# aa5490/Distributed-Training-with-Pipeline-Parallelism

Hardware: AMD Instinct MI355X
Metric: tokens/sec/node + pipeline bubble fraction, GPT-2 PP=1/2/4/8 (GPipe vs 1F1B vs interleaved) (higher is better)
Workload: dtype bf16

## Files before the change

csrc/bindings.cpp:

```cpp
#include <climits>
#include <torch/extension.h>
#include <c10/hip/HIPStream.h>
#include <hip/hip_runtime.h>

#include <algorithm>
#include <cstdint>

extern "C" {
int mp_norm_fwd(int f32, int rms, const void* a, const void* b, const void* w, const void* bias, void* s_out, void* y,
                float* mean, float* rstd, int rows, int D, float eps, float p, uint64_t seed, hipStream_t st);
int mp_norm_bwd(int f32, int rms, const void* dy, const void* s, const void* w, const float* mean, const float* rstd,
                const void* dres, void* ds, void* dbranch, float* dw, float* dbias, float* cs_res, float* cs_ds,
                int rows, int D, float p, uint64_t seed, float* part, hipStream_t st);
int64_t mp_norm_bwd_part_elems(int rows, int D);
int64_t mp_colsum_part_elems(int rows, int cols);
int mp_xent_fwd_bwd(void* logits, const int64_t* target, float* loss, int T, int V, int Vp, float grad_scale,
                    int64_t ignore_index, int write_grad, int f32, hipStream_t st);
int mp_embed_fwd(const int64_t* idx, const void* wte, const void* wpe, void* out, int T, int S, int D, int pos_offset,
                 int f32, hipStream_t st);
int mp_embed_bwd(const int64_t* idx, const void* dout, float* dwte, float* dwpe, int T, int S, int D, int pos_offset,
                 int f32, hipStream_t st);
int mp_sumsq(const float* g, int64_t n, float* out, hipStream_t st);
int mp_scaled_sum(const float* x, int64_t n, float scale, float* out, hipStream_t st);
int mp_gemm_f32(const float* A, const float* B, float* C, const float* bias, int M, int N, int K, int64_t lda,
// ... 35 lines not shown
int mp_doc_bounds(const int64_t* tokens, int64_t eos, int* doc_start, int* doc_end, int B, int S, hipStream_t st);
int mp_attn_decode(const void* q, const void* k, const void* v, const int* lens, void* o, float* ws, int B, int H,
                   int Hkv, int D, int Smax, int max_len, int64_t q_stride, int64_t k_bs, int64_t k_ts, int64_t v_bs,
                   int64_t v_ts, int64_t o_stride, float scale, int splits, hipStream_t st);
int mp_attn_decode_plan(int B, int Hkv, int max_len);
int64_t mp_attn_decode_ws_floats(int B, int H, int D, int splits);
int mp_attn_f32_fwd(const float* q, const float* k, const float* v, float* o, float* lse, int B, int Sq, int Sk, int H,
                    int Hkv, int D, int64_t qs, int64_t ks, int64_t vs, int64_t os, int causal, float scale,
                    float p_drop, uint64_t seed, hipStream_t st);
int mp_attn_f32_bwd(const float* q, const float* k, const float* v, const float* o, const float* dout,
                    const float* lse, float* delta, float* dq, float* dk, float* dv, int B, int Sq, int Sk, int H,
                    int Hkv, int D, int64_t qs, int64_t ks, int64_t vs, int64_t os, int64_t dqs, int64_t dks,
                    int64_t dvs, int causal, float scale, float p_drop, uint64_t seed, hipStream_t st);
int mp_set_drop_step_attn_f32(uint64_t v, hipStream_t st);
int mp_set_drop_step_gemm_f32(uint64_t v, hipStream_t st);
int mp_gemm_f32_set_lanes(int lanes);
int mp_transpose(const void* in, void* out, int R, int C, int64_t ldi, int64_t ldo, hipStream_t st);
int mp_transpose_batched(const void* src, void* dst, const int64_t* desc, const int* tile0, int n, int total_tiles,
                         hipStream_t st);
int mp_set_drop_step_attn(uint64_t v, hipStream_t st);
int mp_set_drop_step_elem(uint64_t v, hipStream_t st);
int mp_set_drop_step_norm(uint64_t v, hipStream_t st);
int mp_set_drop_step_gemm(uint64_t v, hipStream_t st);
int mp_gemm2(const void* A, const void* B, void* C, const void* bias, const void* residual, void* aux, int M, int N,
             int K, int64_t lda, int64_t ldb, int64_t ldc, int64_t ld_res, int64_t ld_aux, int transA, int transB,
             int epilogue, int c_f32_accum, float alpha, int force_cfg, float* ws, float* colsum, float p_drop,
             uint64_t seed, hipStream_t st);
int mp_gemm2_plan(int M, int N, int K, int transA, int transB, int c_f32_accum, int force_cfg, int* split_out);
int64_t mp_gemm2_ws_floats(int cfg, int split, int M, int N, int K);
int mp_gemm2_has_probe_engines();
int mp_gemm_tt_grouped(int n, const void* const* A, const void* const* B, float* const* C, const int* M, const int* N,
                       const int* K, const int64_t* lda, const int64_t* ldb, const int64_t* ldc, float alpha,
                       hipStream_t st);
int mp_probe_spin(unsigned* flag, unsigned expect, int64_t timeout_us, unsigned* result, hipStream_t waiter);
int mp_probe_set(unsigned* flag, unsigned value, hipStream_t setter);
int mp_probe_clock_khz();
int mp_gemm(const void* A, const void* B, void* C, const void* bias, const void* residual, void* aux, int M, int N,
            int K, int64_t lda, int64_t ldb, int64_t ldc, int64_t ld_res, int64_t ld_aux, int transA, int transB,
            int epilogue, int c_f32_accum, float alpha, hipStream_t st);
}

namespace {

hipStream_t cur_stream() { return c10::hip::getCurrentHIPStream().stream(); }

void check(int rc, const char* what) { TORCH_CHECK(rc == 0, "mipipe kernel ", what, " failed with code ", rc); }

const void* ptr_or_null(const c10::optional<torch::Tensor>& t) { return t.has_value() ? t->data_ptr() : nullptr; }

int storage(const torch::Tensor& t, const char* name) {
  TORCH_CHECK(t.scalar_type() == torch::kBFloat16 || t.scalar_type() == torch::kFloat32, name,
              " must be bf16 or f32, got ", t.scalar_type());
  return t.scalar_type() == torch::kFloat32 ? 1 : 0;
}
void* mptr_or_null(const c10::optional<torch::Tensor>& t) { return t.has_value() ? t->data_ptr() : nullptr; }

void req(const torch::Tensor& t, torch::ScalarType dt, const char* name) {
  TORCH_CHECK(t.is_cuda(), name, " must be on the GPU");
  TORCH_CHECK(t.scalar_type() == dt, name, " has wrong dtype ", t.scalar_type());
  TORCH_CHECK(t.is_contiguous(), name, " must be contiguous");
}

void reqn(const torch::Tensor& t, torch::ScalarType dt, int64_t n, const char* name) {
  req(t, dt, name);
  TORCH_CHECK(t.numel() == n, name, " has ", t.numel(), " elements, expected ", n);
}
// ... 544 lines not shown
  }
  if (rc == -2 || rc == -1) return 0;
  check(rc, "gemm2");
  return 1;
}

void gemm_tt_grouped(std::vector<torch::Tensor> dy, std::vector<torch::Tensor> x, std::vector<torch::Tensor> C,
                     double alpha) {
  const int n = (int)dy.size();
  TORCH_CHECK(n == (int)x.size() && n == (int)C.size() && n >= 1 && n <= 8, "gemm_tt_grouped: 1..8 problems");
  const void* A[8];
  const void* B[8];
  float* Cp[8];
  int M[8], N[8], K[8];
  int64_t lda[8], ldb[8], ldc[8];
  for (int i = 0; i < n; ++i) {
    TORCH_CHECK(dy[0].is_cuda(), "gemm_tt_grouped: dy must be on the GPU");
    gemm_operand("gemm_tt_grouped", "dy", dy[i], torch::kBFloat16, dy[0]);
    gemm_operand("gemm_tt_grouped", "x", x[i], torch::kBFloat16, dy[0]);
    gemm_operand("gemm_tt_grouped", "C", C[i], torch::kFloat32, dy[0]);
    TORCH_CHECK(dy[i].size(0) == x[i].size(0) && C[i].size(0) == dy[i].size(1) && C[i].size(1) == x[i].size(1),
                "gemm_tt_grouped: shape mismatch");
    A[i] = dy[i].data_ptr();
    B[i] = x[i].data_ptr();
    Cp[i] = C[i].data_ptr<float>();
    M[i] = (int)dy[i].size(1);
    N[i] = (int)x[i].size(1);
    K[i] = (int)dy[i].size(0);
    lda[i] = dy[i].stride(0);
    ldb[i] = x[i].stride(0);
    ldc[i] = C[i].stride(0);
  }
  check(mp_gemm_tt_grouped(n, A, B, Cp, M, N, K, lda, ldb, ldc, (float)alpha, cur_stream()), "gemm_tt_grouped");
}

void transpose(torch::Tensor in, torch::Tensor out) {
  TORCH_CHECK(in.is_cuda() && out.is_cuda() && in.get_device() == out.get_device(), "transpose: in and out must be on one GPU");
  TORCH_CHECK(in.scalar_type() == torch::kBFloat16 && out.scalar_type() == torch::kBFloat16, "transpose: in and out must be bf16");
  TORCH_CHECK(in.dim() == 2 && out.dim() == 2 && in.stride(1) == 1 && out.stride(1) == 1, "transpose: 2-D rows");
  TORCH_CHECK(in.size(0) > 0 && in.size(1) > 0, "transpose: in is empty");
  TORCH_CHECK(out.size(0) == in.size(1) && out.size(1) == in.size(0), "transpose: shape");
  check(mp_transpose(in.data_ptr(), out.data_ptr(), in.size(0), in.size(1), in.stride(0), out.stride(0),
                     cur_stream()),
        "transpose");
}

void transpose_batched(torch::Tensor src, torch::Tensor dst, torch::Tensor desc, torch::Tensor tile0,
                       int64_t total_tiles) {
  TORCH_CHECK(desc.scalar_type() == torch::kInt64 && tile0.scalar_type() == torch::kInt32 && desc.is_cuda() &&
                  tile0.is_cuda() && desc.size(0) == tile0.size(0),
              "transpose_batched: bad descriptors");
  check(mp_transpose_batched(src.data_ptr(), dst.data_ptr(), desc.data_ptr<int64_t>(), tile0.data_ptr<int>(),
                             (int)desc.size(0), (int)total_tiles, cur_stream()),
        "transpose_batched");
}

int64_t create_stream(int64_t device, int64_t priority) {
  int cur = 0;
  TORCH_CHECK(hipGetDevice(&cur) == hipSuccess, "hipGetDevice");
  TORCH_CHECK(hipSetDevice((int)device) == hipSuccess, "hipSetDevice");
  int lo = 0, hi = 0;
  TORCH_CHECK(hipDeviceGetStreamPriorityRange(&lo, &hi) == hipSuccess, "priority range");
  hipStream_t s = nullptr;
  const hipError_t e = hipStreamCreateWithPriority(&s, hipStreamNonBlocking, priority < 0 ? hi : lo);
  hipSetDevice(cur);
  TORCH_CHECK(e == hipSuccess, "hipStreamCreateWithPriority: ", hipGetErrorString(e));
// ... 131 lines not shown
  m.def("embed_bwd", &embed_bwd);
  m.def("sumsq", &sumsq);
  m.def("scaled_sum", &scaled_sum);
  m.def("zero_", &zero_);
  m.def("gemm_f32", &gemm_f32);
  m.def("gemm_f32_set_lanes", &mp_gemm_f32_set_lanes);
  m.def("gemm_f32_ex", &gemm_f32_ex, pybind11::arg("A"), pybind11::arg("B"), pybind11::arg("C"), pybind11::arg("bias"),
        pybind11::arg("R"), pybind11::arg("X"), pybind11::arg("epi") = 0, pybind11::arg("alpha") = 1.0,
        pybind11::arg("accumulate") = false, pybind11::arg("p_drop") = 0.0, pybind11::arg("seed") = 0,
        pybind11::arg("force_ks") = 0);
  m.def("adamw", &adamw);
  m.def("cast_f32_bf16", &cast_f32_bf16);
  m.def("act_fwd", &act_fwd);
  m.def("act_bwd", &act_bwd);
  m.def("colsum", &colsum);
  m.def("swiglu_fwd", &swiglu_fwd);
  m.def("swiglu_bwd", &swiglu_bwd);
  m.def("rope", &rope);
  m.def("attn_fwd", &attn_fwd);
  m.def("attn_bwd", &attn_bwd);
  m.def("attn_doc_fwd", &attn_doc_fwd);
  m.def("attn_doc_bwd", &attn_doc_bwd);
  m.def("doc_bounds", &doc_bounds);
  m.def("attn_decode", &attn_decode, pybind11::arg("q"), pybind11::arg("k_cache"), pybind11::arg("v_cache"),
        pybind11::arg("lens"), pybind11::arg("o"), pybind11::arg("H"), pybind11::arg("Hkv"), pybind11::arg("D"),
        pybind11::arg("max_len"), pybind11::arg("scale"), pybind11::arg("splits") = 0);
  m.def("attn_decode_plan", [](int64_t B, int64_t Hkv, int64_t max_len) {
    return mp_attn_decode_plan((int)B, (int)Hkv, (int)max_len);
  }, "key splits the decode attention picks for B sequences x Hkv KV heads over max_len keys");
  m.def("gemm", &gemm);
  m.def("lane_merge", &lane_merge, pybind11::arg("g0"), pybind11::arg("lanes"), pybind11::arg("sumsq") = pybind11::none());
  m.def("gemm_tt_grouped", &gemm_tt_grouped, pybind11::arg("dy"), pybind11::arg("x"), pybind11::arg("C"),
        pybind11::arg("alpha") = 1.0);
  m.def("gemm2", &gemm2, pybind11::arg("A"), pybind11::arg("B"), pybind11::arg("C"), pybind11::arg("bias"),
        pybind11::arg("residual"), pybind11::arg("aux"), pybind11::arg("transA"), pybind11::arg("transB"),
        pybind11::arg("epilogue"), pybind11::arg("accum"), pybind11::arg("alpha"), pybind11::arg("force_cfg"),
        pybind11::arg("colsum"), pybind11::arg("p_drop") = 0.0, pybind11::arg("seed") = 0);
  m.def("transpose", &transpose);
  m.def("set_dropout_step", &set_dropout_step);
  m.def("create_stream", &create_stream, pybind11::arg("device"), pybind11::arg("priority") = 0);
  m.def("transpose_batched", &transpose_batched);
  m.def("probe_spin", &probe_spin, pybind11::arg("flag"), pybind11::arg("expect"), pybind11::arg("timeout_us"),
        pybind11::arg("result"), pybind11::arg("waiter") = 0);
  m.def("probe_set", &probe_set, pybind11::arg("flag"), pybind11::arg("value"), pybind11::arg("setter") = 0);
  m.def("probe_clock_khz", []() { return mp_probe_clock_khz(); });
  m.def("gemm2_plan", [](int64_t M, int64_t N, int64_t K, bool transA, bool transB, bool accum, int64_t force_cfg) {
    int split = 1;
    const int cfg = mp_gemm2_plan((int)M, (int)N, (int)K, transA, transB, accum, (int)force_cfg, &split);
    return std::make_tuple(cfg, split);
  }, "engine config + split-K factor the v2 GEMM picks (14: stream-K gemm7)");
  m.def("gemm_f32_plan", [](int64_t M, int64_t N, int64_t K, int64_t force_ks) {
    int split = 1, sk_grid = 0, sk_chunk = 0;
    const int big = mp_gemm_f32_plan((int)M, (int)N, (int)K, (int)force_ks, &split, &sk_grid, &sk_chunk);
    return std::make_tuple(big != 0, split, sk_grid, sk_chunk);
  }, "what gemm_f32_ex will run: (128x128 engine, split-K factor, stream-K workgroups, K-tile pairs per workgroup)");
  m.def("gemm2_has_probe_engines", []() { return mp_gemm2_has_probe_engines() != 0; });
}
```

csrc/kernels/gemm2.hip:

```cpp
#include "mp_common.h"

using namespace mp;

typedef __attribute__((ext_vector_type(4))) short s16x4;
typedef __attribute__((ext_vector_type(8))) short s16x8;

#ifndef MP_G3_GROUP
#define MP_G3_GROUP 2
#endif
#ifndef MP_G2_GROUP
#define MP_G2_GROUP 8
#endif

#ifndef MP_G4_SR
#define MP_G4_SR 2
#endif

#ifndef MP_GROUP_MAX
#define MP_GROUP_MAX 8
#endif

namespace g2 {

enum Epi { EPI_NONE = 0, EPI_BIAS = 1, EPI_BIAS_GELU = 2, EPI_BIAS_RELU = 3, EPI_BIAS_RES = 4, EPI_RES = 5,
           EPI_DGELU = 6, EPI_DRELU = 7 };

constexpr int BK = 64;
constexpr int NT = 512;

__device__ __forceinline__ int swz8(int row) { return (((row >> 1) & 1) << 2) | ((row >> 2) & 3); }
__device__ __forceinline__ int swz16(int row) { return ((row & 3) << 2) | ((row >> 2) & 3); }
__device__ __forceinline__ int swzq(int row) { return (((row >> 1) & 7) + 6) & 7; }
// ... 518 lines not shown
        for (int j = 0; j < TN; ++j) bfr[1][j] = frag16<TB, BN>(sbB, wn + 16 * j, 1);
      }
      __builtin_amdgcn_sched_barrier(0);
      __builtin_amdgcn_s_setprio(1);
#pragma unroll
      for (int i = 0; i < TM; ++i)
#pragma unroll
        for (int j = 0; j < TN; ++j) acc[i][j] = mfma16(af[s][i], bfr[s][j], acc[i][j]);
      __builtin_amdgcn_s_setprio(0);
      __builtin_amdgcn_sched_barrier(0);
    }
    }
    asm volatile("s_waitcnt lgkmcnt(0)" ::: "memory");
    __builtin_amdgcn_s_barrier();
    asm volatile("" ::: "memory");
    if (t + 2 < nk) {
      issue(t & 1, t + 2);
      wait_vmcnt<PW>();
    } else {
      wait_vmcnt<0>();
    }
    asm volatile("" ::: "memory");
    __builtin_amdgcn_s_barrier();
    asm volatile("" ::: "memory");
  }

  epilogue<BM, BN, WM, WN, EPI, ACC>(Stage16<TM, TN>{acc, wn, lane}, smem, m0, n0, wr, Cv, bias, R, AUX, WS, M, N, ldc,
                                     ldr, ldx, alpha, nsplit, p_drop, seed);
  }

}


template <int EPI, bool ACC, bool M16, bool TT = false>
__global__ void __launch_bounds__(NT, 1) __attribute__((amdgpu_waves_per_eu(2, 2)))
gemm3_kernel(const bf16_t* __restrict__ A, const bf16_t* __restrict__ B, void* __restrict__ Cv,
             const bf16_t* __restrict__ bias, const bf16_t* __restrict__ R, bf16_t* __restrict__ AUX,
             float* __restrict__ WS, int M, int N, int K, int64_t lda, int64_t ldb, int64_t ldc, int64_t ldr,
             int64_t ldx, float alpha, float p_drop, uint64_t seed, int tile_lim) {
  if (p_drop > 0.f) seed = step_seed(seed);
  constexpr int BM = 256, BN = 256, WM = 2, WN = 4;
  constexpr int HALF = 128 * 128;
  constexpr int BUF = 4 * HALF;
  extern __shared__ __attribute__((aligned(16))) char smem[];

  const int gm = (M + BM - 1) / BM, gn = (N + BN - 1) / BN;
  const int nwg = tile_lim > 0 ? tile_lim : gm * gn;
  int wg, split;
  if (gridDim.y > 1 && tile_lim == 0) {
    const int v = xcd_remap((int)blockIdx.x + (int)gridDim.x * (int)blockIdx.y, nwg * (int)gridDim.y);
    split = v / nwg;
    wg = v % nwg;
  } else {
    wg = xcd_remap((int)blockIdx.x, nwg);
    split = (int)blockIdx.y;
  }
  constexpr int GROUP = MP_G3_GROUP;
  const int group = wg / (GROUP * gn);
  const int first_m = group * GROUP;
  const int gsz = min(gm - first_m, GROUP);
  const int tm = tile_lim > 0 ? wg / gn : first_m + (wg % (GROUP * gn)) % gsz;
  const int tn = tile_lim > 0 ? wg % gn : (wg % (GROUP * gn)) / gsz;
  const int m0 = tm * BM, n0 = tn * BN;

  const int lane = threadIdx.x & 63, hl = lane >> 5, l32 = lane & 31;
  const int wave = __builtin_amdgcn_readfirstlane(threadIdx.x >> 6);
  const int wr = wave / WN, wc = wave % WN;
  const int wm = wr * (BM / WM), wn = wc * (BN / WN);

  const int nsplit = gridDim.y;
  const int ktiles = K / BK;
  const int kt0 = split * ktiles / nsplit;
  const int nk = (split + 1) * ktiles / nsplit - kt0;

  static_assert(!TT || M16, "the TT build exists with 16x16x32 MFMAs only");
  const int lr = lane >> 3;
  const int lc = (lane & 7) ^ (M16 ? swzq(8 * (wave & 1) + lr) : swz8(8 * (wave & 1) + lr));
  const bf16_t* pa[2];
  const bf16_t* pb[2];
  const bf16_t* ta1[2];
  const bf16_t* tb1[2];
  if constexpr (TT) {
    const int kr = lane >> 4;
    const int ic = 8 * ((lane & 15) ^ ((kr << 2) | (wave & 3)));
    const int am = ic < 64 ? ic : ic + 64, bn = 64 * (ic >> 5) + (ic & 31);
    auto cm = [&](int m) { return m < M ? m : M - 8; };
    auto cn = [&](int n) { return n < N ? n : N - 8; };
#pragma unroll
    for (int j = 0; j < 2; ++j) {
      const int64_t krow = (int64_t)kt0 * BK + 4 * wave + 32 * j + kr;
      pa[j] = A + krow * lda + cm(m0 + am);
      ta1[j] = A + krow * lda + cm(m0 + am + 64);
      pb[j] = B + krow * ldb + cn(n0 + bn);
      tb1[j] = B + krow * ldb + cn(n0 + bn + 32);
    }
  }
#pragma unroll
  for (int j = 0; j < 2 && !TT; ++j) {
    int ra = m0 + 128 * j + 8 * wave + lr;
    ra = ra < M ? ra : M - 1;
    int rb = n0 + 64 * ((wave >> 2) + 2 * j) + 8 * (wave & 3) + lr;
    rb = rb < N ? rb : N - 1;
    pa[j] = A + (int64_t)ra * lda + (int64_t)kt0 * BK + lc * 8;
// ... 187 lines not shown
#pragma unroll
      for (int j = 0; j < 2; ++j) b1[j][s_] = fq(buf + 3 * HALF, rB + 16 * j, s_);
    if (t + 1 < nk) issue(3, t + 1);
    if (steady) wait_vmcnt<8>(); else wait_vmcnt<0>();
    G3_BAR();
    asm volatile("s_waitcnt lgkmcnt(0)" ::: "memory");
    G4_MFMA(0, b1, 2);
    G3_BAR();
#pragma unroll
    for (int s_ = 0; s_ < 2; ++s_)
#pragma unroll
      for (int i = 0; i < 4; ++i) af[i][s_] = fq(buf + HALF, rA + 16 * i, s_);
    if (steady) issue(0, t + 2);
    G3_BAR();
    asm volatile("s_waitcnt lgkmcnt(0)" ::: "memory");
    G4_MFMA(4, b0, 0);
    G3_BAR();
    if (steady) {
      issue(1, t + 2);
      wait_vmcnt<8>();
    } else {
      wait_vmcnt<0>();
    }
    G3_BAR();
    G4_MFMA(4, b1, 2);
    G3_BAR();
  }
#undef G4_MFMA
#undef G3_BAR
  if (wr == 0) __builtin_amdgcn_s_barrier();
  __syncthreads();
  epilogue<BM, BN, WM, WN, EPI, ACC>(Stage16<8, 4>{acc, wn, lane}, smem, m0, n0, wr, Cv, bias, R, AUX, WS, M, N, ldc,
                                     ldr, ldx, alpha, nsplit, p_drop, seed, nullptr, 0, 0, split);
  }
}

template <int EPI, bool ACC, bool M16, bool TT = false>
static int launch3(const void* A, const void* B, void* C, const void* bias, const void* R, void* X, float* ws, int M,
                   int N, int K,
                   int64_t lda, int64_t ldb, int64_t ldc, int64_t ldr, int64_t ldx, float alpha, int split,
                   float p_drop, uint64_t seed, hipStream_t st, int tile_lim = 0) {
  constexpr int LDS_MAIN = 2 * 4 * 128 * 128;
  constexpr int EPI_BYTES = 128 * (256 + 4) * 4;
  constexpr int LDS = LDS_MAIN > EPI_BYTES ? LDS_MAIN : EPI_BYTES;
  auto kern = gemm3_kernel<EPI, ACC, M16, TT>;
  static bool attr = false;
  if (!attr) {
    hipFuncSetAttribute((const void*)kern, hipFuncAttributeMaxDynamicSharedMemorySize, LDS);
    attr = true;
  }
  const int nwg = tile_lim > 0 ? tile_lim : ((M + 255) / 256) * ((N + 255) / 256);
  static const bool split_remap = [] {
    const char* e = getenv("MIPIPE_G3_SPLIT_REMAP");
    return e && e[0] == '1';
  }();
  if (tile_lim == 0 && !split_remap) tile_lim = -1;
  kern<<<dim3(nwg, split), NT, LDS, st>>>((const bf16_t*)A, (const bf16_t*)B, C, (const bf16_t*)bias,
                                          (const bf16_t*)R, (bf16_t*)X, ws, M, N, K, lda, ldb, ldc, ldr, ldx, alpha, p_drop, seed,
                                          tile_lim);
  return (int)hipGetLastError();
}

template <int EPI, bool ACC>
__global__ void __launch_bounds__(NT, 1) __attribute__((amdgpu_waves_per_eu(2, 2)))
gemm6_kernel(const bf16_t* __restrict__ A, const bf16_t* __restrict__ B, void* __restrict__ Cv,
             const bf16_t* __restrict__ bias, const bf16_t* __restrict__ R, bf16_t* __restrict__ AUX,
// ... 1270 lines not shown
  int best = 3, best_split = 1;
  float best_t = 3.0e38f;
  const int kt = K / BK;
  for (int c = 0; c < 4; ++c) {
    const int cus = 256;
    const int slots = c == 3 ? 2 * cus : cus;
    if (outer && CFGS[c].bn == 192) continue;
    const int tiles = ((M + CFGS[c].bm - 1) / CFGS[c].bm) * ((N + CFGS[c].bn - 1) / CFGS[c].bn);
    const float area = (float)(CFGS[c].bm * CFGS[c].bn) / (256.f * 256.f) * (c == 3 ? 2.f : 1.f);
    static const int acc_cap = [] {
      const char* e = getenv("MIPIPE_DW_MAXSPLIT");
      const int v = e ? atoi(e) : 32;
      return v > 0 ? v : 32;
    }();
    const int acc_max = kt / 4 < acc_cap ? kt / 4 : acc_cap;
    const int max_split = acc ? acc_max : (kt / 3 < 8 ? kt / 3 : 8);
    for (int s = 1; s <= (max_split > 1 ? max_split : 1); ++s) {
      const int work = tiles * s;
      const int rounds = (work + slots - 1) / slots;
      const int kper = (kt + s - 1) / s;
      const float epi = s > 1 ? (acc ? 6.f : 8.f) : 2.f;
      const float t = rounds * (kper + epi + 2.f) * area / CFGS[c].eff;
      if (t < best_t * 0.999f) {
        best_t = t;
        best = c;
        best_split = s;
      }
    }
  }
  *split_out = best_split;
  return best;
}

}

using namespace g2;

template <bool TA, bool TB, int EPI, bool ACC>
static int dispatch(int cfg, const void* A, const void* B, void* C, const void* bias, const void* R, void* X, float* ws,
                    int M,
                    int N, int K, int64_t lda, int64_t ldb, int64_t ldc, int64_t ldr, int64_t ldx, float alpha,
                    int split, float p_drop, uint64_t seed, hipStream_t st) {
  if constexpr (TA && TB && ACC && EPI == EPI_NONE) {
    if (cfg == 13) return launchs<64, 64, EPI, ACC, true, true>(A, B, C, bias, R, X, ws, M, N, K, lda, ldb, ldc, ldr, ldx, alpha, split, p_drop, seed, st);
    if (cfg == 6) return launch3<EPI, ACC, true, true>(A, B, C, bias, R, X, ws, M, N, K, lda, ldb, ldc, ldr, ldx, alpha, split, p_drop, seed, st);
  }
  if constexpr (!TA && !TB) {
    if (cfg == 10) return launchs<64, 64, EPI, ACC>(A, B, C, bias, R, X, ws, M, N, K, lda, ldb, ldc, ldr, ldx, alpha, split, p_drop, seed, st);
    if (cfg == 11) return launchs<64, 32, EPI, ACC>(A, B, C, bias, R, X, ws, M, N, K, lda, ldb, ldc, ldr, ldx, alpha, split, p_drop, seed, st);
    if (cfg == 12) return launchs<32, 32, EPI, ACC>(A, B, C, bias, R, X, ws, M, N, K, lda, ldb, ldc, ldr, ldx, alpha, split, p_drop, seed, st);
    if (cfg == 4) return launch3<EPI, ACC, false>(A, B, C, bias, R, X, ws, M, N, K, lda, ldb, ldc, ldr, ldx, alpha, split, p_drop, seed, st);
    if (cfg == 5) return launch3<EPI, ACC, true>(A, B, C, bias, R, X, ws, M, N, K, lda, ldb, ldc, ldr, ldx, alpha, split, p_drop, seed, st);
    if (cfg == 9) return launch6<EPI, ACC>(A, B, C, bias, R, X, ws, M, N, K, lda, ldb, ldc, ldr, ldx, alpha, p_drop, seed, st);
    if (cfg == 15) return launch8<EPI, ACC, 2>(A, B, C, bias, R, X, ws, M, N, K, lda, ldb, ldc, ldr, ldx, alpha, p_drop, seed, st);
    if (cfg == 16) return launch8<EPI, ACC, 3>(A, B, C, bias, R, X, ws, M, N, K, lda, ldb, ldc, ldr, ldx, alpha, p_drop, seed, st);
#ifdef MP_PROBE_ENGINES
    if constexpr (!ACC) {
      if (cfg == 8) return launch5<EPI>(A, B, C, bias, R, X, ws, M, N, K, lda, ldb, ldc, ldr, ldx, alpha, p_drop, seed, st);
    }
#endif
  }
  switch (cfg) {
    case 0: return launch<256, 256, 2, 4, TA, TB, EPI, ACC>(A, B, C, bias, R, X, ws, M, N, K, lda, ldb, ldc, ldr, ldx, alpha, split, p_drop, seed, st);
    case 1: return launch<256, 192, 4, 2, TA, TB, EPI, ACC>(A, B, C, bias, R, X, ws, M, N, K, lda, ldb, ldc, ldr, ldx, alpha, split, p_drop, seed, st);
    case 2: return launch<256, 128, 4, 2, TA, TB, EPI, ACC>(A, B, C, bias, R, X, ws, M, N, K, lda, ldb, ldc, ldr, ldx, alpha, split, p_drop, seed, st);
    default: return launch<128, 128, 2, 4, TA, TB, EPI, ACC>(A, B, C, bias, R, X, ws, M, N, K, lda, ldb, ldc, ldr, ldx, alpha, split, p_drop, seed, st);
// ... 267 lines not shown
                                  const int64_t* ldc, float alpha, hipStream_t st) {
  if (n <= 0) return 0;
  if (n > MP_GROUP_MAX) return -1;
  GroupTT g{};
  g.n = n;
  g.alpha = alpha;
  int t = 0;
  for (int i = 0; i < n; ++i) {
    if (M[i] % 8 || N[i] % 8 || K[i] % BK || M[i] <= 0 || N[i] <= 0) return -1;
    g.A[i] = (const bf16_t*)A[i];
    g.B[i] = (const bf16_t*)B[i];
    g.C[i] = C[i];
    g.M[i] = M[i];
    g.N[i] = N[i];
    g.K[i] = K[i];
    g.lda[i] = lda[i];
    g.ldb[i] = ldb[i];
    g.ldc[i] = ldc[i];
    g.tile_start[i] = t;
    t += ((M[i] + 63) / 64) * ((N[i] + 63) / 64);
  }
  for (int i = n; i <= MP_GROUP_MAX; ++i) g.tile_start[i] = t;
  constexpr int STAGE = (64 + 64) * BK * 2;
  constexpr int EPI_BYTES = 32 * (64 + 4) * 4;
  constexpr int LDS = 2 * STAGE > EPI_BYTES ? 2 * STAGE : EPI_BYTES;
  static bool attr = false;
  if (!attr) {
    hipFuncSetAttribute((const void*)gemms_tt_grouped_kernel, hipFuncAttributeMaxDynamicSharedMemorySize, LDS);
    attr = true;
  }
  gemms_tt_grouped_kernel<<<t, 256, LDS, st>>>(g);
  return (int)hipGetLastError();
}
```

distributed-training-with-pipeline-parallelism_amd/models/native.py:

```python
from __future__ import annotations

import contextlib
import hashlib
import os
import math
from dataclasses import dataclass
from typing import Callable, Dict, List, Optional, Sequence, Tuple

import torch

from .. import ops
from .config import NativeConfig



@dataclass
class ParamSpec:
    name: str
    shape: Tuple[int, ...]
    init: str
    decay: bool
    std: float = 0.02
    transpose: bool = False

# ... 426 lines not shown
                wjobs.append(ops.DW(dy, gact, self.g("ffn.w2.weight")))
                if cfg.bias and not fuse_b1:
                    wjobs.append(lambda da=da: ops.colsum(da, self.g("ffn.w1.bias")))
                wjobs.append(ops.DW(da, h2, self.g("ffn.w1.weight")))
                dh2 = ops.linear_dx(da, self.w("ffn.w1.weight"), wt=self.wt("ffn.w1.weight"))
            fuse_cs = cfg.bias and kind == "layernorm"
            dx2, _ = ops.norm_bwd(dh2, st["x2"], self.w("ffn_norm.weight"), st["mu2"], st["rs2"], kind=kind,
                                  dres=dy, dw=self.g("ffn_norm.weight"), dbias=self.gb("ffn_norm.bias"),
                                  colsum_dres=self.g("ffn.w2.bias") if fuse_cs else None,
                                  colsum_ds=self.g("attn.wo.bias") if fuse_cs else None)
            if cfg.bias and not fuse_cs:
                wjobs.append(lambda dy=dy: ops.colsum(dy, self.g("ffn.w2.bias")))
            o = st["o"]
            do = ops.linear_dx(dx2, self.w("attn.wo.weight"), wt=self.wt("attn.wo.weight"))
            wjobs.append(ops.DW(dx2, o, self.g("attn.wo.weight")))
            if cfg.bias and not fuse_cs:
                wjobs.append(lambda dx2=dx2: ops.colsum(dx2, self.g("attn.wo.bias")))
            qkv = st["qkv"]
            q, k, v = qkv[:, : H * Dh], qkv[:, H * Dh:(H + KV) * Dh], qkv[:, (H + KV) * Dh:]
            dqkv = torch.empty_like(qkv)
            dq, dk, dv = dqkv[:, : H * Dh], dqkv[:, H * Dh:(H + KV) * Dh], dqkv[:, (H + KV) * Dh:]
            docs = ctx.docs
            fuse_qkv_bias = cfg.bias and cfg.pos != "rope" and _FUSE_QKV_BIAS and docs is None
            ops.attn_bwd(q, k, v, o, do, st["lse"], dq, dk, dv, B, S, S, H, KV, Dh, cfg.causal,
                         p_drop=cfg.dropout, seed=_seed(sd, 1),
                         dbias=self.g("attn.wqkv.bias") if fuse_qkv_bias else None,
                         doc_start=docs[0] if docs is not None else None,
                         doc_end=docs[1] if docs is not None else None)
            if cfg.pos == "rope":
                ops.rope_(dqkv, self.rope[0], self.rope[1], S, H, KV, Dh, inverse=True)
            h1 = st["h1"]
            wjobs.append(ops.DW(dqkv, h1, self.g("attn.wqkv.weight")))
            if cfg.bias and not fuse_qkv_bias:
                wjobs.append(lambda dqkv=dqkv: ops.colsum(dqkv, self.g("attn.wqkv.bias")))
            dh1 = ops.linear_dx(dqkv, self.w("attn.wqkv.weight"), wt=self.wt("attn.wqkv.weight"))
            dx, _ = ops.norm_bwd(dh1, st["x"], self.w("attn_norm.weight"), st["mu1"], st["rs1"], kind=kind,
                                 dres=dx2, dw=self.g("attn_norm.weight"), dbias=self.gb("attn_norm.bias"))
        if ov is not None:
            ov.run(wjobs)
        elif weight_grads:
            ops.run_wjobs(wjobs)
        else:
            defer.extend(wjobs)
        del ctx.layers[self.i]
        return dx

    def _mha(self, prefix, xq, xkv, B, S, seed, st, key, self_attn: bool):
        cfg = self.cfg
        H, Dh, d = cfg.n_heads, cfg.head_dim, cfg.d_model
        W, b = self.w(prefix + ".in_proj_weight"), self.w(prefix + ".in_proj_bias")
        if self_attn:
            qkv, _ = ops.linear(xq, W, b)
            q, k, v = qkv[:, :d], qkv[:, d:2 * d], qkv[:, 2 * d:]
            st[key + "qkv"] = qkv
        else:
            q, _ = ops.linear(xq, W[:d], b[:d])
            kv, _ = ops.linear(xkv, W[d:], b[d:])
            k, v = kv[:, :d], kv[:, d:]
            st[key + "q"], st[key + "kv"] = q, kv
        o = torch.empty(xq.shape[0], d, device=xq.device, dtype=xq.dtype)
        lse = torch.empty(B * H * S, device=xq.device, dtype=torch.float32)
        ops.attn_fwd(q, k, v, o, lse, B, S, S, H, H, Dh, False, p_drop=cfg.dropout, seed=seed)
        st[key + "o"], st[key + "lse"] = o, lse
        out, _ = ops.linear(o, self.w(prefix + ".out_proj.weight"), self.w(prefix + ".out_proj.bias"))
        return out

    def _ref_forward(self, h, B, S, st, sd):
# ... 404 lines not shown
```

distributed-training-with-pipeline-parallelism_amd/ops/kernels.py:

```python
from __future__ import annotations

import importlib.util
import math
import os
from typing import Optional, Tuple

import torch

_PKG_DIR = os.path.dirname(os.path.dirname(os.path.abspath(__file__)))
_EXT = None
_EXT_ERR: Optional[str] = None

ACT = {"none": 0, "gelu_tanh": 1, "gelu": 1, "relu": 2}
EPI_NONE, EPI_BIAS, EPI_BIAS_GELU, EPI_BIAS_RELU, EPI_BIAS_RES, EPI_RES, EPI_DGELU, EPI_DRELU = range(8)
LOG2E = 1.4426950408889634

GEMM_BACKEND = os.environ.get("MIPIPE_GEMM", "hip")
_PLAIN_BEST: dict = {}


def _plain_pick(key, run_hip, run_lib) -> str:
    if GEMM_BACKEND != "auto":
        return GEMM_BACKEND
    d = _PLAIN_BEST.get(key)
# ... 492 lines not shown
class F32MultiheadAttention(torch.nn.MultiheadAttention):

    def forward(self, query, key, value, key_padding_mask=None, need_weights=True, attn_mask=None,
                average_attn_weights=True, is_causal=False):
        stock = (need_weights or key_padding_mask is not None or attn_mask is not None or not query.is_cuda
                 or query.dtype != torch.float32 or not self._qkv_same_embed_dim or self.bias_k is not None
                 or self.add_zero_attn or query.dim() != 3)
        if stock:
            return super().forward(query, key, value, key_padding_mask=key_padding_mask, need_weights=need_weights,
                                   attn_mask=attn_mask, average_attn_weights=average_attn_weights, is_causal=is_causal)
        return _mha_projected(self, query, key, value, is_causal, _LinearF32.apply), None


_F32_SWAP = {torch.nn.Linear: F32Linear, torch.nn.modules.linear.NonDynamicallyQuantizableLinear: F32Linear,
             torch.nn.MultiheadAttention: F32MultiheadAttention}


def use_f32_kernels(module: torch.nn.Module, on: bool = True) -> int:
    n = 0
    for mod in module.modules():
        if on:
            cls = _F32_SWAP.get(type(mod))
            if cls is not None:
                mod._mipipe_f32_orig_cls = type(mod)
                mod.__class__ = cls
                n += 1
        elif type(mod) in (F32Linear, F32MultiheadAttention):
            mod.__class__ = mod.__dict__.pop("_mipipe_f32_orig_cls")
            n += 1
    return n


_WGRAD_GROUP = os.environ.get("MIPIPE_WGRAD_GROUP", "1") != "0"
_GROUP_MAX = 8


class DW:
    __slots__ = ("dy", "x", "dw", "alpha")

    def __init__(self, dy: torch.Tensor, x: torch.Tensor, dw: torch.Tensor, alpha: float = 1.0):
        self.dy, self.x, self.dw, self.alpha = dy, x, dw, alpha

    def __call__(self):
        linear_dw(self.dy, self.x, self.dw, self.alpha)

    def groupable(self) -> bool:
        dy, x, dw = self.dy, self.x, self.dw
        if not (_gpu(dy) and dy.dtype == torch.bfloat16 and x.dtype == torch.bfloat16 and dw.dtype == torch.float32):
            return False
        if dy.stride(1) != 1 or x.stride(1) != 1 or dw.stride(1) != 1:
            return False
        T, N = dy.shape
        K = x.shape[1]
        if T % 64 or N % 8 or K % 8 or T > 4096:
            return False
        return ((N + 255) // 256) * ((K + 255) // 256) < 64


def run_wjobs(jobs) -> None:
    if not jobs:
        return
    rest, groups = [], {}
    if _WGRAD_GROUP and GEMM_BACKEND != "blas":
        for j in jobs:
            if isinstance(j, DW) and j.groupable():
                groups.setdefault(j.alpha, []).append(j)
            else:
                rest.append(j)
    else:
        rest = list(jobs)
    for alpha, g in groups.items():
        if len(g) == 1:
            g[0]()
            continue
        for i in range(0, len(g), _GROUP_MAX):
            part = g[i:i + _GROUP_MAX]
            _ext().gemm_tt_grouped([j.dy for j in part], [j.x for j in part], [j.dw for j in part], float(alpha))
    for j in rest:
        j()


def act_fwd(a: torch.Tensor, act: str, p_drop: float = 0.0, seed: int = 0, out=None):
    if out is None:
        out = torch.empty_like(a)
    if _gpu(a):
        _ext().act_fwd(a, out, ACT[act], float(p_drop), int(seed))
        return out
    y = _act_cpu(a.float(), act)
    if p_drop > 0:
        y = y * _cpu_dropout_mask(a.shape, p_drop, seed, a.device)
    out.copy_(y.to(out.dtype))
    return out


def act_bwd(dg: torch.Tensor, a: torch.Tensor, act: str, dbias: Optional[torch.Tensor] = None,
            p_drop: float = 0.0, seed: int = 0, out=None, saved: str = "pre"):
    if saved not in ("pre", "grad"):
        raise ValueError(f"saved must be 'pre' or 'grad', not {saved!r}")
    if out is None:
        out = torch.empty_like(dg)
    if saved == "grad":
        d = dg.float() * a.float()
        if p_drop > 0:
            if _gpu(dg):
                raise ValueError("the dropout mask with a saved derivative is fused into linear_dx's epilogue")
            d = d * _cpu_dropout_mask(a.shape, p_drop, seed, a.device)
        out.copy_(d.to(out.dtype))
        if dbias is not None:
            if _gpu(dg):
                _ext().colsum(out, dbias)
# ... 310 lines not shown
```

Measured before the change: 1.012 million.

## Add grouped split-K weight-gradient GEMM for long-token DW jobs

Adds a grouped TT GEMM kernel built on the gemm3 256x256 tile path. It packs several weight-gradient problems that share a large token count into one launch, with split-K picked to fill the device and a grouped reduction afterwards. Weight-gradient jobs with T >= 16384 and fewer than 256 tiles are batched this way instead of launched one by one, which targets poor CU occupancy on small-output, long-K GEMMs. The cost is a workspace allocation per call, an extra reduction pass, and a refactor of the gemm3 kernel into a shared device tile function.

```diff
diff --git a/csrc/bindings.cpp b/csrc/bindings.cpp
--- a/csrc/bindings.cpp
+++ b/csrc/bindings.cpp
@@ -91,6 +91,10 @@
 int mp_gemm_tt_grouped(int n, const void* const* A, const void* const* B, float* const* C, const int* M, const int* N,
                        const int* K, const int64_t* lda, const int64_t* ldb, const int64_t* ldc, float alpha,
                        hipStream_t st);
+int mp_gemm3_tt_grouped_plan(int n, const int* M, const int* N, int K, int force_split, int64_t* ws_floats);
+int mp_gemm3_tt_grouped(int n, const void* const* A, const void* const* B, float* const* C, const int* M, const int* N,
+                        int K, const int64_t* lda, const int64_t* ldb, const int64_t* ldc, float alpha, int S, float* ws,
+                        hipStream_t st);
 int mp_probe_spin(unsigned* flag, unsigned expect, int64_t timeout_us, unsigned* result, hipStream_t waiter);
 int mp_probe_set(unsigned* flag, unsigned value, hipStream_t setter);
 int mp_probe_clock_khz();
@@ -701,6 +705,50 @@
     ldc[i] = C[i].stride(0);
   }
   check(mp_gemm_tt_grouped(n, A, B, Cp, M, N, K, lda, ldb, ldc, (float)alpha, cur_stream()), "gemm_tt_grouped");
+}
+
+int64_t gemm_dw_grouped(std::vector<torch::Tensor> dy, std::vector<torch::Tensor> x, std::vector<torch::Tensor> C,
+                        double alpha, int64_t split) {
+  const char* fn = "gemm_dw_grouped";
+  const int n = (int)dy.size();
+  TORCH_CHECK(n == (int)x.size() && n == (int)C.size() && n >= 1 && n <= 8, fn, ": 1..8 problems");
+  TORCH_CHECK(split >= 0 && split <= INT_MAX, fn, ": split ", split, " must be >= 0");
+  const void* A[8];
+  const void* B[8];
+  float* Cp[8];
+  int M[8], N[8];
+  int64_t lda[8], ldb[8], ldc[8];
+  TORCH_CHECK(dy[0].is_cuda(), fn, ": dy must be on the GPU");
+  const int64_t T = dy[0].dim() == 2 ? dy[0].size(0) : 0;
+  for (int i = 0; i < n; ++i) {
+    gemm_operand(fn, "dy", dy[i], torch::kBFloat16, dy[0]);
+    gemm_operand(fn, "x", x[i], torch::kBFloat16, dy[0]);
+    gemm_operand(fn, "C", C[i], torch::kFloat32, dy[0]);
+    TORCH_CHECK(dy[i].size(0) == T && x[i].size(0) == T, fn, ": every dy and x needs the same token count T = ", T,
+                ", problem ", i, " has ", dy[i].size(0), " and ", x[i].size(0));
+    TORCH_CHECK(C[i].size(0) == dy[i].size(1) && C[i].size(1) == x[i].size(1), fn, ": C[", i, "] must be [",
+                dy[i].size(1), ", ", x[i].size(1), "]");
+    TORCH_CHECK(dy[i].size(1) % 8 == 0 && x[i].size(1) % 8 == 0, fn, ": problem ", i, ": M = ", dy[i].size(1),
+                " and N = ", x[i].size(1), " must be multiples of 8");
+    TORCH_CHECK(dy[i].size(1) <= INT_MAX && x[i].size(1) <= INT_MAX, fn, ": M, N must fit 32 bits");
+    A[i] = dy[i].data_ptr();
+    B[i] = x[i].data_ptr();
+    Cp[i] = C[i].data_ptr<float>();
+    M[i] = (int)dy[i].size(1);
+    N[i] = (int)x[i].size(1);
+    lda[i] = dy[i].stride(0);
+    ldb[i] = x[i].stride(0);
+    ldc[i] = C[i].stride(0);
+  }
+  TORCH_CHECK(T % 64 == 0 && T <= INT_MAX, fn, ": T = ", T, " must be a multiple of 64");
+  int64_t ws_n = 0;
+  const int S = mp_gemm3_tt_grouped_plan(n, M, N, (int)T, (int)split, &ws_n);
+  torch::Tensor ws;
+  if (ws_n > 0) ws = torch::empty({ws_n}, C[0].options().dtype(torch::kFloat32));
+  check(mp_gemm3_tt_grouped(n, A, B, Cp, M, N, (int)T, lda, ldb, ldc, (float)alpha, S,
+                            ws.defined() ? ws.data_ptr<float>() : nullptr, cur_stream()),
+        fn);
+  return S;
 }
 
 void transpose(torch::Tensor in, torch::Tensor out) {
@@ -898,6 +946,8 @@
   m.def("lane_merge", &lane_merge, pybind11::arg("g0"), pybind11::arg("lanes"), pybind11::arg("sumsq") = pybind11::none());
   m.def("gemm_tt_grouped", &gemm_tt_grouped, pybind11::arg("dy"), pybind11::arg("x"), pybind11::arg("C"),
         pybind11::arg("alpha") = 1.0);
+  m.def("gemm_dw_grouped", &gemm_dw_grouped, pybind11::arg("dy"), pybind11::arg("x"), pybind11::arg("C"),
+        pybind11::arg("alpha") = 1.0, pybind11::arg("split") = 0);
   m.def("gemm2", &gemm2, pybind11::arg("A"), pybind11::arg("B"), pybind11::arg("C"), pybind11::arg("bias"),
         pybind11::arg("residual"), pybind11::arg("aux"), pybind11::arg("transA"), pybind11::arg("transB"),
         pybind11::arg("epilogue"), pybind11::arg("accum"), pybind11::arg("alpha"), pybind11::arg("force_cfg"),
diff --git a/csrc/kernels/gemm2.hip b/csrc/kernels/gemm2.hip
--- a/csrc/kernels/gemm2.hip
+++ b/csrc/kernels/gemm2.hip
@@ -1,3 +1,5 @@
+#include <climits>
+
 #include "mp_common.h"
 
 using namespace mp;
@@ -582,29 +584,18 @@
 }
 
 
-template <int EPI, bool ACC, bool M16, bool TT = false>
-__global__ void __launch_bounds__(NT, 1) __attribute__((amdgpu_waves_per_eu(2, 2)))
-gemm3_kernel(const bf16_t* __restrict__ A, const bf16_t* __restrict__ B, void* __restrict__ Cv,
-             const bf16_t* __restrict__ bias, const bf16_t* __restrict__ R, bf16_t* __restrict__ AUX,
-             float* __restrict__ WS, int M, int N, int K, int64_t lda, int64_t ldb, int64_t ldc, int64_t ldr,
-             int64_t ldx, float alpha, float p_drop, uint64_t seed, int tile_lim) {
-  if (p_drop > 0.f) seed = step_seed(seed);
+template <int EPI, bool ACC, bool M16, bool TT>
+__device__ __forceinline__ void gemm3_tile(char* smem, const bf16_t* __restrict__ A, const bf16_t* __restrict__ B,
+                                           void* __restrict__ Cv, const bf16_t* __restrict__ bias,
+                                           const bf16_t* __restrict__ R, bf16_t* __restrict__ AUX,
+                                           float* __restrict__ WS, int M, int N, int K, int64_t lda, int64_t ldb,
+                                           int64_t ldc, int64_t ldr, int64_t ldx, float alpha, float p_drop,
+                                           uint64_t seed, int tile_lim, int wg, int split, int nsplit) {
   constexpr int BM = 256, BN = 256, WM = 2, WN = 4;
   constexpr int HALF = 128 * 128;
   constexpr int BUF = 4 * HALF;
-  extern __shared__ __attribute__((aligned(16))) char smem[];
 
   const int gm = (M + BM - 1) / BM, gn = (N + BN - 1) / BN;
-  const int nwg = tile_lim > 0 ? tile_lim : gm * gn;
-  int wg, split;
-  if (gridDim.y > 1 && tile_lim == 0) {
-    const int v = xcd_remap((int)blockIdx.x + (int)gridDim.x * (int)blockIdx.y, nwg * (int)gridDim.y);
-    split = v / nwg;
-    wg = v % nwg;
-  } else {
-    wg = xcd_remap((int)blockIdx.x, nwg);
-    split = (int)blockIdx.y;
-  }
   constexpr int GROUP = MP_G3_GROUP;
   const int group = wg / (GROUP * gn);
   const int first_m = group * GROUP;
@@ -618,7 +609,6 @@
   const int wr = wave / WN, wc = wave % WN;
   const int wm = wr * (BM / WM), wn = wc * (BN / WN);
 
-  const int nsplit = gridDim.y;
   const int ktiles = K / BK;
   const int kt0 = split * ktiles / nsplit;
   const int nk = (split + 1) * ktiles / nsplit - kt0;
@@ -872,6 +862,81 @@
   __syncthreads();
   epilogue<BM, BN, WM, WN, EPI, ACC>(Stage16<8, 4>{acc, wn, lane}, smem, m0, n0, wr, Cv, bias, R, AUX, WS, M, N, ldc,
                                      ldr, ldx, alpha, nsplit, p_drop, seed, nullptr, 0, 0, split);
+  }
+}
+
+template <int EPI, bool ACC, bool M16, bool TT = false>
+__global__ void __launch_bounds__(NT, 1) __attribute__((amdgpu_waves_per_eu(2, 2)))
+gemm3_kernel(const bf16_t* __restrict__ A, const bf16_t* __restrict__ B, void* __restrict__ Cv,
+             const bf16_t* __restrict__ bias, const bf16_t* __restrict__ R, bf16_t* __restrict__ AUX,
+             float* __restrict__ WS, int M, int N, int K, int64_t lda, int64_t ldb, int64_t ldc, int64_t ldr,
+             int64_t ldx, float alpha, float p_drop, uint64_t seed, int tile_lim) {
+  if (p_drop > 0.f) seed = step_seed(seed);
+  extern __shared__ __attribute__((aligned(16))) char smem[];
+  const int nwg = tile_lim > 0 ? tile_lim : ((M + 255) / 256) * ((N + 255) / 256);
+  int wg, split;
+  if (gridDim.y > 1 && tile_lim == 0) {
+    const int v = xcd_remap((int)blockIdx.x + (int)gridDim.x * (int)blockIdx.y, nwg * (int)gridDim.y);
+    split = v / nwg;
+    wg = v % nwg;
+  } else {
+    wg = xcd_remap((int)blockIdx.x, nwg);
+    split = (int)blockIdx.y;
+  }
+  gemm3_tile<EPI, ACC, M16, TT>(smem, A, B, Cv, bias, R, AUX, WS, M, N, K, lda, ldb, ldc, ldr, ldx, alpha, p_drop, seed,
+                                tile_lim, wg, split, (int)gridDim.y);
+}
+
+struct GroupTT3 {
+  const bf16_t* A[MP_GROUP_MAX];
+  const bf16_t* B[MP_GROUP_MAX];
+  float* C[MP_GROUP_MAX];
+  int64_t lda[MP_GROUP_MAX], ldb[MP_GROUP_MAX], ldc[MP_GROUP_MAX];
+  int64_t elem_start[MP_GROUP_MAX + 1];
+  int M[MP_GROUP_MAX], N[MP_GROUP_MAX];
+  int tile_start[MP_GROUP_MAX + 1];
+  int n, K, S;
+  float alpha;
+  float* ws;
+};
+
+__global__ void __launch_bounds__(NT, 1) __attribute__((amdgpu_waves_per_eu(2, 2)))
+gemm3_tt_grouped_kernel(const GroupTT3 g) {
+  extern __shared__ __attribute__((aligned(16))) char smem[];
+  const int total = g.tile_start[g.n];
+  const int v = xcd_remap((int)blockIdx.x, total * g.S);
+  int p = 0;
+#pragma unroll
+  for (int i = 1; i < MP_GROUP_MAX; ++i)
+    if (i < g.n && v >= g.tile_start[i] * g.S) p = i;
+  const int tiles = g.tile_start[p + 1] - g.tile_start[p];
+  const int local = v - g.tile_start[p] * g.S;
+  const int split = local / tiles, wg = local % tiles;
+  float* ws = g.S > 1 ? g.ws + g.elem_start[p] * g.S : nullptr;
+  gemm3_tile<EPI_NONE, true, true, true>(smem, g.A[p], g.B[p], g.C[p], nullptr, nullptr, nullptr, ws, g.M[p], g.N[p],
+                                         g.K, g.lda[p], g.ldb[p], g.ldc[p], 0, 0, g.alpha, 0.f, 0, 0, wg, split, g.S);
+}
+
+__global__ void __launch_bounds__(256) splitk_reduce_grouped_kernel(const GroupTT3 g) {
+  const int64_t n4 = g.elem_start[g.n] / 4;
+  for (int64_t i = (int64_t)blockIdx.x * 256 + threadIdx.x; i < n4; i += (int64_t)gridDim.x * 256) {
+    const int64_t e = i * 4;
+    int p = 0;
+#pragma unroll
+    for (int j = 1; j < MP_GROUP_MAX; ++j)
+      if (j < g.n && e >= g.elem_start[j]) p = j;
+    const int64_t le = e - g.elem_start[p], slab = (int64_t)g.M[p] * g.N[p];
+    const float* w = g.ws + g.elem_start[p] * g.S + le;
+    const int m = (int)(le / g.N[p]), n = (int)(le % g.N[p]);
+    float4 acc = *reinterpret_cast<const float4*>(w);
+    for (int s = 1; s < g.S; ++s) {
+      const float4 t = *reinterpret_cast<const float4*>(w + s * slab);
+      acc.x += t.x; acc.y += t.y; acc.z += t.z; acc.w += t.w;
+    }
+    float4* cp = reinterpret_cast<float4*>(g.C[p] + (int64_t)m * g.ldc[p] + n);
+    float4 c = *cp;
+    c.x += acc.x; c.y += acc.y; c.z += acc.z; c.w += acc.w;
+    *cp = c;
   }
 }
 
@@ -2208,6 +2273,33 @@
   return best;
 }
 
+static int choose_group_split(int tiles, int kt, int force) {
+  static const int env_force = [] {
+    const char* e = getenv("MIPIPE_DW_GROUP_SPLIT");
+    return e ? atoi(e) : 0;
+  }();
+  static const int cap = [] {
+    const char* e = getenv("MIPIPE_DW_MAXSPLIT");
+    const int v = e ? atoi(e) : 32;
+    return v > 0 ? v : 32;
+  }();
+  if (force <= 0) force = env_force;
+  if (force > 0) return force < kt ? force : (kt > 0 ? kt : 1);
+  const int smax = kt / 4 < cap ? kt / 4 : cap;
+  int best = 1;
+  float best_fill = 0.f;
+  for (int s = 1; s <= (smax > 1 ? smax : 1); ++s) {
+    const int work = tiles * s, rounds = (work + 255) / 256;
+    const float fill = (float)work / (float)(rounds * 256);
+    if (fill >= 0.8f) return s;
+    if (fill > best_fill) {
+      best_fill = fill;
+      best = s;
+    }
+  }
+  return best;
+}
+
 }
 
 using namespace g2;
@@ -2541,3 +2633,67 @@
   gemms_tt_grouped_kernel<<<t, 256, LDS, st>>>(g);
   return (int)hipGetLastError();
 }
+
+extern "C" int mp_gemm3_tt_grouped_plan(int n, const int* M, const int* N, int K, int force_split,
+                                        int64_t* ws_floats) {
+  int tiles = 0;
+  int64_t elems = 0;
+  for (int i = 0; i < n; ++i) {
+    tiles += ((M[i] + 255) / 256) * ((N[i] + 255) / 256);
+    elems += (int64_t)M[i] * N[i];
+  }
+  const int S = choose_group_split(tiles, K / BK, force_split);
+  *ws_floats = S > 1 ? (int64_t)S * elems : 0;
+  return S;
+}
+
+extern "C" int mp_gemm3_tt_grouped(int n, const void* const* A, const void* const* B, float* const* C, const int* M,
+                                   const int* N, int K, const int64_t* lda, const int64_t* ldb, const int64_t* ldc,
+                                   float alpha, int S, float* ws, hipStream_t st) {
+  if (n <= 0) return 0;
+  if (n > MP_GROUP_MAX || K <= 0 || K % BK || S < 1 || S > K / BK || (S > 1 && ws == nullptr)) return -1;
+  GroupTT3 g{};
+  g.n = n;
+  g.K = K;
+  g.S = S;
+  g.alpha = alpha;
+  g.ws = ws;
+  int t = 0;
+  int64_t e = 0;
+  for (int i = 0; i < n; ++i) {
+    if (M[i] % 8 || N[i] % 8 || M[i] <= 0 || N[i] <= 0) return -1;
+    g.A[i] = (const bf16_t*)A[i];
+    g.B[i] = (const bf16_t*)B[i];
+    g.C[i] = C[i];
+    g.M[i] = M[i];
+    g.N[i] = N[i];
+    g.lda[i] = lda[i];
+    g.ldb[i] = ldb[i];
+    g.ldc[i] = ldc[i];
+    g.tile_start[i] = t;
+    g.elem_start[i] = e;
+    t += ((M[i] + 255) / 256) * ((N[i] + 255) / 256);
+    e += (int64_t)M[i] * N[i];
+  }
+  for (int i = n; i <= MP_GROUP_MAX; ++i) {
+    g.tile_start[i] = t;
+    g.elem_start[i] = e;
+  }
+  if ((int64_t)t * S > INT_MAX) return -1;
+  constexpr int LDS_MAIN = 2 * 4 * 128 * 128;
+  constexpr int EPI_BYTES = 128 * (256 + 4) * 4;
+  constexpr int LDS = LDS_MAIN > EPI_BYTES ? LDS_MAIN : EPI_BYTES;
+  static bool attr = false;
+  if (!attr) {
+    hipFuncSetAttribute((const void*)gemm3_tt_grouped_kernel, hipFuncAttributeMaxDynamicSharedMemorySize, LDS);
+    attr = true;
+  }
+  gemm3_tt_grouped_kernel<<<t * S, NT, LDS, st>>>(g);
+  int rc = (int)hipGetLastError();
+  if (rc == 0 && S > 1) {
+    const int blocks = (int)std::min<int64_t>((e / 4 + 255) / 256, 4096);
+    splitk_reduce_grouped_kernel<<<blocks, 256, 0, st>>>(g);
+    rc = (int)hipGetLastError();
+  }
+  return rc;
+}
diff --git a/distributed-training-with-pipeline-parallelism_amd/models/native.py b/distributed-training-with-pipeline-parallelism_amd/models/native.py
--- a/distributed-training-with-pipeline-parallelism_amd/models/native.py
+++ b/distributed-training-with-pipeline-parallelism_amd/models/native.py
@@ -482,7 +482,7 @@
             h1 = st["h1"]
             wjobs.append(ops.DW(dqkv, h1, self.g("attn.wqkv.weight")))
             if cfg.bias and not fuse_qkv_bias:
-                wjobs.append(lambda dqkv=dqkv: ops.colsum(dqkv, self.g("attn.wqkv.bias")))
+                wjobs.append(ops.ColSum(dqkv, self.g("attn.wqkv.bias")))
             dh1 = ops.linear_dx(dqkv, self.w("attn.wqkv.weight"), wt=self.wt("attn.wqkv.weight"))
             dx, _ = ops.norm_bwd(dh1, st["x"], self.w("attn_norm.weight"), st["mu1"], st["rs1"], kind=kind,
                                  dres=dx2, dw=self.g("attn_norm.weight"), dbias=self.gb("attn_norm.bias"))
diff --git a/distributed-training-with-pipeline-parallelism_amd/ops/kernels.py b/distributed-training-with-pipeline-parallelism_amd/ops/kernels.py
--- a/distributed-training-with-pipeline-parallelism_amd/ops/kernels.py
+++ b/distributed-training-with-pipeline-parallelism_amd/ops/kernels.py
@@ -548,7 +548,9 @@
 
 
 _WGRAD_GROUP = os.environ.get("MIPIPE_WGRAD_GROUP", "1") != "0"
+_WGRAD_GROUP3 = os.environ.get("MIPIPE_WGRAD_GROUP3", "1") != "0"
 _GROUP_MAX = 8
+_GROUP3_MIN_T = 16384
 
 
 class DW:
@@ -560,38 +562,73 @@
     def __call__(self):
         linear_dw(self.dy, self.x, self.dw, self.alpha)
 
-    def groupable(self) -> bool:
+    def _tt_operands(self) -> bool:
         dy, x, dw = self.dy, self.x, self.dw
         if not (_gpu(dy) and dy.dtype == torch.bfloat16 and x.dtype == torch.bfloat16 and dw.dtype == torch.float32):
+            return False
+        if dy.dim() != 2 or x.dim() != 2 or dw.dim() != 2:
             return False
         if dy.stride(1) != 1 or x.stride(1) != 1 or dw.stride(1) != 1:
             return False
         T, N = dy.shape
-        K = x.shape[1]
-        if T % 64 or N % 8 or K % 8 or T > 4096:
-            return False
-        return ((N + 255) // 256) * ((K + 255) // 256) < 64
+        return not (T % 64 or N % 8 or x.shape[1] % 8)
+
+    def tiles256(self) -> int:
+        return ((self.dy.shape[1] + 255) // 256) * ((self.x.shape[1] + 255) // 256)
+
+    def groupable(self) -> bool:
+        return self._tt_operands() and self.dy.shape[0] <= 4096 and self.tiles256() < 64
+
+    def groupable3(self) -> bool:
+        return self._tt_operands() and self.dy.shape[0] >= _GROUP3_MIN_T and self.tiles256() < 256
+
+
+class ColSum:
+    __slots__ = ("x", "dbias")
+
+    def __init__(self, x: torch.Tensor, dbias: torch.Tensor):
+        self.x, self.dbias = x, dbias
+
+    def __call__(self):
+        colsum(self.x, self.dbias)
+
+
+def plan_wjobs(jobs):
+    small, long_ = [], []
+    if not (_WGRAD_GROUP and GEMM_BACKEND != "blas"):
+        return small, long_, list(jobs)
+    sg, lg = {}, {}
+    for j in jobs:
+        if _WGRAD_GROUP3 and isinstance(j, DW) and j.groupable3():
+            lg.setdefault((j.alpha, j.dy.shape[0]), []).append(j)
+        elif isinstance(j, DW) and j.groupable():
+            sg.setdefault(j.alpha, []).append(j)
+    for g in sg.values():
+        if len(g) > 1:
+            small.extend(g[i:i + _GROUP_MAX] for i in range(0, len(g), _GROUP_MAX))
+    for g in lg.values():
+        parts = [g[i:i + _GROUP_MAX] for i in range(0, len(g), _GROUP_MAX)]
+        long_.extend(part for part in parts if len(part) > 1)
+    grouped = {id(j) for part in small + long_ for j in part}
+    return small, long_, [j for j in jobs if id(j) not in grouped]
+
+
+def _run_group_small(part) -> None:
+    _ext().gemm_tt_grouped([j.dy for j in part], [j.x for j in part], [j.dw for j in part], float(part[0].alpha))
+
+
+def _run_group_long(part) -> None:
+    _ext().gemm_dw_grouped([j.dy for j in part], [j.x for j in part], [j.dw for j in part], float(part[0].alpha))
 
 
 def run_wjobs(jobs) -> None:
     if not jobs:
         return
-    rest, groups = [], {}
-    if _WGRAD_GROUP and GEMM_BACKEND != "blas":
-        for j in jobs:
-            if isinstance(j, DW) and j.groupable():
-                groups.setdefault(j.alpha, []).append(j)
-            else:
-                rest.append(j)
-    else:
-        rest = list(jobs)
-    for alpha, g in groups.items():
-        if len(g) == 1:
-            g[0]()
-            continue
-        for i in range(0, len(g), _GROUP_MAX):
-            part = g[i:i + _GROUP_MAX]
-            _ext().gemm_tt_grouped([j.dy for j in part], [j.x for j in part], [j.dw for j in part], float(alpha))
+    small, long_, rest = plan_wjobs(jobs)
+    for part in small:
+        _run_group_small(part)
+    for part in long_:
+        _run_group_long(part)
     for j in rest:
         j()
 
```

After: 1.066 million (median of 6 runs). 5.3% higher.
